# KangWelly/Assignment-for-AAE6102_GNSS-SDR

Measured on NVIDIA B200. Metric: search cells/s (PRN x Doppler x code-phase), 32-PRN acquisition, higher is better.
Workload: dtype f32

## Files before the change

### assignment-for-aae6102_gnss-sdr_b200/csrc/gnss_engine.h

```cpp
#pragma once
#include "gnss_radix.h"

#if defined(__CUDACC__)
#include <cuda_runtime.h>
#else
#include <cmath>
#endif

namespace gnss {

template <int Q>
struct Geo {
    static constexpr int N = 2000 * Q;
    static constexpr int ROW = 125 * Q;
    static constexpr int NX = 16 * (2 * Q - 1) * 125;
    static constexpr int M1 = 125 * Q, M2 = 16 * Q, M3 = 2000;
    static constexpr int INV1 = cmodinv(M1 % 16, 16);
    static constexpr int INV2 = cmodinv(M2 % 125, 125);
    static constexpr int INV3 = cmodinv(M3 % Q, Q);
    static constexpr int E1 = M1 * INV1, E2 = M2 * INV2, E3 = M3 * INV3;
    static_assert(Q % 2 == 1 && Q % 5 != 0, "Q must be coprime to 2000");
    static_assert(INV1 && INV2 && INV3, "no modular inverse");

    GNSS_HD static int good(int a, int b, int c) { return (a * M1 + b * M2 + c * M3) % N; }
// ... 193 lines not shown
    using X = GeoX<Q>;
    const int al = task / (5 * Q);
    const cf* p = D + task * 25 + al * (S::RS - S::ROW);
    cf v[25];
    static_for<0, 25>([&](auto ic) {
        constexpr int I = decltype(ic)::value;
        v[I] = p[I];
    });
    dft25(v);
    cf* q = xrow0 + al * X::RSX + (task - al * X::NT);
    static_for<0, 25>([&](auto ic) {
        constexpr int I = decltype(ic)::value;
        q[I * X::NTP] = v[5 * (I % 5) + I / 5];
    });
}
template <int Q, int R, class Storer>
GNSS_HD void pass4_task_xt(int j, int rank, const cf* __restrict__ X, Storer& st) {
    using GX = GeoX<Q>;
    using SX = SplitX<Q, R>;
    const int t = 2 * j;
    const int e = rank * SX::CHX + t;
    if (t >= SX::CHX || e >= GX::RSX) return;
    cf w0[16], w1[16];
    static_for<0, 16>([&](auto ac) {
        constexpr int Aidx = decltype(ac)::value;
        const cf2 v = ld_cg2(reinterpret_cast<const cf2*>(X + Aidx * GX::RSX + e));
        w0[Aidx] = v.lo;
        w1[Aidx] = v.hi;
    });
    dft16(w0);
    dft16(w1);
    st.template store2x<Q, R>(t, w0, w1);
}

template <int Q, int R, class Storer>
GNSS_HD void pass4_task(int j, int rank, cf* const* Dall, Storer& st) {
    using S = Split<Q, R>;
    const int t = 2 * j;
    const int col = rank * S::CH + t;
    if (t >= S::CH || col >= S::ROW) return;
    cf w0[16], w1[16];
    static_for<0, 16>([&](auto ac) {
        constexpr int Aidx = decltype(ac)::value;
        const cf2 v = *reinterpret_cast<const cf2*>(Dall[Aidx / S::A] + (Aidx % S::A) * S::RS + col);
        w0[Aidx] = v.lo;
        w1[Aidx] = v.hi;
    });
// ... 91 lines not shown
};

struct RegAccumStorer {
    float (&a0)[16];
    float (&a1)[16];
    template <int Q, int R>
    GNSS_HD void store2x(int , const cf (&w0)[16], const cf (&w1)[16]) {
        static_for<0, 16>([&](auto i_) {
            constexpr int I = decltype(i_)::value;
            constexpr int AP = (I / 4) + 4 * (I % 4);
            a0[AP] = cnorm_acc(w0[I], a0[AP]);
            a1[AP] = cnorm_acc(w1[I], a1[AP]);
        });
    }
};

struct SpectrumStorer {
    cf* __restrict__ out;
    float scale;
    int conj;
    int extended;
    template <int Q, int R>
    GNSS_HD void store1(int col, const cf (&w)[16]) {
        using G = Geo<Q>;
        const int cp = col / 125, pos = col - cp * 125;
        const int bp = G::bprime_of_pos(pos);
        const int bg = (bp * G::INV2) % 125, cg = (cp * G::INV3) % Q;
        const int planes = extended ? 2 * Q - 1 : Q;
        static_for<0, 16>([&](auto i_) {
            constexpr int I = decltype(i_)::value;
// ... 149 lines not shown
```

### assignment-for-aae6102_gnss-sdr_b200/csrc/gnss_internal.h

```cpp
#pragma once
#include <cuda_runtime.h>
#include <cstddef>
#include <cstdint>
#include "gnss_engine.h"

namespace gnss {

struct Candidate {
    float peak;
    int lag;
    double sum_all;
    double sum_win;
};

struct SearchArgs {
    const cf* cc;
    const cf* x;
    const int* bin_base;
    const int* bin_shift;
    int P, B, K;
    int row_first, n_rows;
    int w;
    Candidate* cand;
    int cand_stride;
    float* surface;
    cf* scratch;
    unsigned* group_ctr;
    Candidate* row_slots;
    float* partial;
    unsigned* part_ctr;
    unsigned* row_ticket;
    int row_granular;
#ifdef GNSS_TIMELINE
    unsigned long long* timeline;
#endif
};

struct WipeArgs {
    const void* raw;
    int data_type, precision, coh_ms, K;
    size_t block_bytes;
    const double* base_freq_hz;
    double fs_hz;
    const double* means;
    cf* x;
};

// ... 56 lines not shown
```

### assignment-for-aae6102_gnss-sdr_b200/csrc/gnss_kernels.cuh

```cuda
#pragma once
#include <cooperative_groups.h>
#include <climits>
#include "gnss_internal.h"

namespace gnss {
namespace cg = cooperative_groups;

struct NaturalLoader {
    static constexpr bool kStreams = false;
    const cf* __restrict__ in;
    template <int Q>
    __device__ __forceinline__ void load(int a, int b, cf (&z)[Q]) const {
        static_for<0, Q>([&](auto c_) {
            constexpr int C = decltype(c_)::value;
            z[C] = in[Geo<Q>::good(a, b, C)];
        });
    }
};
struct NaturalStorer {
    cf* __restrict__ out;
    template <int Q, int R>
    __device__ __forceinline__ void store2(int col, int, const cf (&w0)[16], const cf (&w1)[16]) {
        static_for<0, 16>([&](auto i_) {
            constexpr int I = decltype(i_)::value;
// ... 516 lines not shown
        }
        if constexpr (R > 1) cluster.sync(); else __syncthreads();
    }
}

__device__ __forceinline__ void group_arrive(unsigned* ctr) {
#ifdef GNSS_EXPERIMENT_NOFENCE
    asm volatile("red.relaxed.gpu.global.add.u32 [%0], 1;" ::"l"(ctr) : "memory");
#else
    asm volatile("red.release.gpu.global.add.u32 [%0], 1;" ::"l"(ctr) : "memory");
#endif
}
__device__ __forceinline__ void group_arrive_n(unsigned* ctr, unsigned n) {
    asm volatile("red.release.gpu.global.add.u32 [%0], %1;" ::"l"(ctr), "r"(n) : "memory");
}
__device__ __forceinline__ void group_spin(const unsigned* ctr, unsigned target) {
    unsigned v;
    do {
        asm volatile("ld.acquire.gpu.global.u32 %0, [%1];" : "=r"(v) : "l"(ctr) : "memory");
    } while ((int)(v - target) < 0);
}

template <int Q, int R, int T>
__device__ __noinline__ void publish_plane(float* acc, float* dst, int tid) {
    using SX = SplitX<Q, R>;
    for (int j = tid; j < SX::P4_TASKS; j += T) {
#pragma unroll
        for (int ap = 0; ap < 16; ++ap) {
            float2* p = reinterpret_cast<float2*>(acc + ap * SX::CHX + 2 * j);
            __stcg(reinterpret_cast<float2*>(dst + ap * SX::CHX + 2 * j), *p);
            *p = make_float2(0.f, 0.f);
        }
    }
}
template <int Q, int R, int T>
__device__ __noinline__ void merge_planes(float* acc, const float* planes, int n_planes, int tid) {
// ... 42 lines not shown
    using SX = SplitX<Q, R>;
    const int tid = threadIdx.x;
    const int tid2 = (tid + T - 32) % T;
    const int tid3 = (tid + T - (64 % T)) % T;
    const int rank = blockIdx.x % R, group = blockIdx.x / R, ngroups = gridDim.x / R;
    extern __shared__ __align__(16) unsigned char smem_raw[];
    cf* D = reinterpret_cast<cf*>(smem_raw);
    float* acc = reinterpret_cast<float*>(D + S::D_ELEMS);
    Tw4* tw = reinterpret_cast<Tw4*>(acc + Smem<Q, R>::acc_floats);
    RedScratch* rs = reinterpret_cast<RedScratch*>(tw + 100);
    constexpr size_t XBUF = (size_t)16 * GX::RSX;
    cf* xch = a.scratch + (size_t)group * 2 * XBUF;
    unsigned* ctr = a.group_ctr + group;
    Candidate* slots = a.row_slots + (size_t)group * R;
    unsigned target = 0;
    fill_tw125(tw, tid, T);
    constexpr bool kRoomy = (T * MINB <= 512);
    constexpr bool kRegAcc = (Q <= 13) && kRoomy && (SX::P4_TASKS <= T);
    float racc0[16], racc1[16];
#pragma unroll
    for (int q = 0; q < 16; ++q) { racc0[q] = 0.f; racc1[q] = 0.f; }
    RegAccumStorer rst{racc0, racc1};
    PowerAccumStorer st{acc};
    auto dump_acc = [&]() {
        if constexpr (kRegAcc) {
            if (tid < SX::P4_TASKS) {
#pragma unroll
                for (int ap = 0; ap < 16; ++ap) {
                    *reinterpret_cast<float2*>(acc + ap * SX::CHX + 2 * tid) = make_float2(racc0[ap], racc1[ap]);
                    racc0[ap] = 0.f; racc1[ap] = 0.f;
                }
            }
        }
    };
    const int n_rows = a.n_rows;
    auto loader_of = [&](int lrow) {
        const int row = a.row_first + lrow;
        const int p = row % a.P, b = row / a.P;
        int sa, sb, sc;
        G::shift_coords(a.bin_shift[b], sa, sb, sc);
        return SearchLoader{a.cc + (size_t)p * G::N, a.x + (size_t)a.bin_base[b] * a.K * G::NX, sa, sb, sc};
    };
    const int full = n_rows / ngroups, tail_base = full * ngroups, n_tail = n_rows - tail_base;
    auto tb = [&](int g) -> int {
        return a.row_granular ? (g < n_tail ? g : n_tail) * a.K : (int)((unsigned)g * (unsigned)(n_tail * a.K) / (unsigned)ngroups);
    };
    struct Part { int row, kb, ke; };
    auto part = [&](int i) -> Part {
        if (i < full) return Part{i * ngroups + group, 0, a.K};
        const int t0 = tb(group), t1 = tb(group + 1), r0 = t0 / a.K, e0 = min(t1, (r0 + 1) * a.K);
        if (i == full) return Part{tail_base + r0, t0 - r0 * a.K, e0 - r0 * a.K};
        return Part{tail_base + r0 + 1, 0, t1 - e0};
    };
    auto count_parts = [&]() -> int {
        const int t0 = tb(group), t1 = tb(group + 1);
        return full + (t0 < t1 ? 1 + (min(t1, (t0 / a.K + 1) * a.K) < t1) : 0);
    };
    if (count_parts() == 0) return;
    int i = 0, par = 0;
    const Part first = part(0);
    int left = first.ke - first.kb;
    bool later = first.kb > 0;
    for (int e = tid; e < SX::ACC_ELEMS; e += T) acc[e] = 0.f;
    SearchLoader ld = loader_of(first.row);
    ld.x += (size_t)first.kb * G::NX;
    for (int t = tid; t < S::P1_TASKS; t += T) pass1_task<Q, R>(t, rank, ld, D);
    __syncthreads();
    pass2_all<Q, R, T>(D, tw, tid2);
    __syncthreads();
    for (int t = tid3; t < S::P3_TASKS; t += T) pass3_task_xt<Q, R>(t, D, xch + (size_t)rank * S::A * GX::RSX);
#ifdef GNSS_TIMELINE
    int tl_iter = 0;
#endif
    for (;;) {
#ifdef GNSS_TIMELINE
        ++tl_iter;
#endif
        GNSS_TL(0);
        const bool last_of_part = (left == 1);
        const bool more = !last_of_part || i + 1 < count_parts();
        const cf* buf = xch + (size_t)par * XBUF;
        cf* nbuf = xch + (size_t)(par ^ 1) * XBUF;
        par ^= 1;
        target += R;
        if (more) {
            if (last_of_part) {
                const Part np = part(i + 1);
                ld = loader_of(np.row);
                ld.x += (size_t)np.kb * G::NX;
            } else {
                ld.x += G::NX;
            }
            cf z[Q];
            const bool has = tid < S::P1_TASKS;
            if (has) pass1_compute<Q, R>(tid, rank, ld, z);
            constexpr bool kTwo = (Q <= 13) && kRoomy && (S::P1_TASKS > T) && (S::P1_TASKS <= 2 * T);
            cf z2[kTwo ? Q : 1];
            const bool has2 = kTwo && tid + T < S::P1_TASKS;
            if constexpr (kTwo) { if (has2) pass1_compute<Q, R>(tid + T, rank, ld, z2); }
            GNSS_TL(1);
            GNSS_KSYNC();
            GNSS_TL(2);
            if (tid == 0) group_arrive(ctr);
            GNSS_TL(3);
            if (has) pass1_store<Q, R>(tid, z, D);
            if constexpr (kTwo) {
                if (has2) pass1_store<Q, R>(tid + T, z2, D);
            } else if constexpr (S::P1_TASKS > T) {
                for (int t = tid + T; t < S::P1_TASKS; t += T) pass1_task<Q, R>(t, rank, ld, D);
            }
            GNSS_TL(4);
            GNSS_KSYNC();
            GNSS_TL(5);
            pass2_all<Q, R, T>(D, tw, tid2);
            GNSS_TL(6);
        } else {
            GNSS_KSYNC();
            if (tid == 0) group_arrive(ctr);
        }
#ifndef GNSS_EXPERIMENT_NOSPIN
        if (tid == 0) group_spin(ctr, target);
#endif
        GNSS_TL(7);
        GNSS_KSYNC();
        GNSS_TL(8);
#pragma unroll 1
        for (int half = 0; half < 2; ++half) {
            const int flip = (((tid >> 5) + 1) >> 1) & 1;
            if ((half ^ flip) == 0) {
                if constexpr (kRegAcc) {
                    if (tid < SX::P4_TASKS) pass4_task_xt<Q, R>(tid, rank, buf, rst);
                } else {
                    for (int t = tid; t < SX::P4_TASKS; t += T) pass4_task_xt<Q, R>(t, rank, buf, st);
                }
            } else if (more) {
                for (int t = tid3; t < S::P3_TASKS; t += T) pass3_task_xt<Q, R>(t, D, nbuf + (size_t)rank * S::A * GX::RSX);
            }
        }
        GNSS_TL(10);
        if (later) {
            const Part cp = part(i);
            const int kk = cp.ke - left;
            int gf = group - 1;
            while (tb(gf) > (cp.row - tail_base) * a.K) --gf;
            float* dst = a.partial + (((size_t)gf * (a.K - 1) + (kk - 1)) * R + rank) * SX::ACC_ELEMS;
            dump_acc();
            publish_plane<Q, R, T>(acc, dst, tid);
            if (last_of_part) {
                __syncthreads();
                if (tid == 0) group_arrive_n(a.part_ctr + (size_t)gf * R + rank, (unsigned)(cp.ke - cp.kb));
            }
        } else if (last_of_part) {
            dump_acc();
            __syncthreads();
            const Part cp = part(i);
            const int row = cp.row;
            if (cp.ke < a.K) {
                if (tid == 0) group_spin(a.part_ctr + (size_t)group * R + rank, (unsigned)(a.K - cp.ke));
                __syncthreads();
                merge_planes<Q, R, T>(acc, a.partial + (((size_t)group * (a.K - 1) + (cp.ke - 1)) * R + rank) * SX::ACC_ELEMS,
                                      a.K - cp.ke, tid);
                __syncthreads();
            }
            const int p = (a.row_first + row) % a.P, b = (a.row_first + row) / a.P;
            float bv = -1.f;
            int bm = INT_MAX;
            double ss = 0.0;
            if (a.surface) {
                for (int e = tid; e < SX::ACC_ELEMS; e += T) {
                    const int ap = e / SX::CHX, t = e - ap * SX::CHX;
                    const int ex = rank * SX::CHX + t;
                    if (GX::valid(ex)) {
                        const float v = acc[e];
                        const int m = GX::lag_of(ap, ex);
// ... 17 lines not shown
                            const int ex = rank * SX::CHX + t;
                            if (vv[u] >= bv && GX::valid(ex)) {
                                const int m = GX::lag_of(ap, ex);
                                if (peak_better(vv[u], m, bv, bm)) { bv = vv[u]; bm = m; }
                            }
                        }
                    }
                }
            }
            block_reduce<T>(bv, bm, ss, rs);
            target += R;
            if (tid == 0) {
                Candidate c; c.peak = bv; c.lag = bm; c.sum_all = ss; c.sum_win = 0.0;
                slots[rank] = c;
                group_arrive(ctr);
                group_spin(ctr, target);
                float gv = -1.f;
                int gm = INT_MAX;
                for (int r = 0; r < R; ++r) {
                    const float ov = __ldcg(&slots[r].peak);
                    const int om = __ldcg(&slots[r].lag);
                    if (peak_better(ov, om, gv, gm)) { gv = ov; gm = om; }
                }
                rs->g_peak = gv;
                rs->g_lag = gm;
            }
            __syncthreads();
            const int gm = rs->g_lag;
            double wsum = 0.0;
            for (int i = tid; i < 2 * a.w - 1; i += T) {
                const int m = gm - (a.w - 1) + i;
                if (m >= 0 && m < G::N) {
                    int ap, ex;
                    GX::cell_of_lag(m, ap, ex);
                    if (ex / SX::CHX == rank) {
                        const float v = acc[ap * SX::CHX + (ex - rank * SX::CHX)];
                        wsum += (double)v * (double)v;
                    }
                }
            }
            float dv = -1.f;
            int dm = INT_MAX;
            block_reduce<T>(dv, dm, wsum, rs);
            if constexpr (!kRegAcc)
                for (int e = tid; e < SX::ACC_ELEMS; e += T) acc[e] = 0.f;
            if (tid == 0) {
                slots[rank].sum_win = wsum;
                unsigned old;
                asm volatile("atom.acq_rel.gpu.global.add.u32 %0, [%1], 1;" : "=r"(old) : "l"(a.row_ticket + group) : "memory");
                if ((old + 1) % R == 0) {
                    double s_all = 0.0, s_win = 0.0;
                    for (int r = 0; r < R; ++r) {
                        s_all += __ldcg(&slots[r].sum_all);
                        s_win += __ldcg(&slots[r].sum_win);
                    }
                    Candidate c;
                    c.peak = rs->g_peak;
                    c.lag = rs->g_lag;
                    c.sum_all = s_all;
                    c.sum_win = s_win;
                    a.cand[(size_t)p * a.cand_stride + b] = c;
                }
            }
        }
        if (!more) break;
        if (last_of_part) {
            const Part np = part(++i);
            left = np.ke - np.kb;
            later = np.kb > 0;
        } else {
            --left;
        }
    }
}

template <class K, class A>
static cudaError_t launch_clustered(K kern, const A& args, int units, int R, int T, size_t smem, cudaStream_t s) {
    cudaLaunchConfig_t cfg = {};
    cfg.gridDim = dim3((unsigned)(units * R), 1, 1);
    cfg.blockDim = dim3((unsigned)T, 1, 1);
    cfg.dynamicSmemBytes = smem;
    cfg.stream = s;
    cudaLaunchAttribute attr[1];
    attr[0].id = cudaLaunchAttributeClusterDimension;
    attr[0].val.clusterDim.x = (unsigned)R;
    attr[0].val.clusterDim.y = 1;
    attr[0].val.clusterDim.z = 1;
    cfg.attrs = attr;
// ... 19 lines not shown
        if (e != cudaSuccess) return e;
        e = cudaFuncSetAttribute(fine_kernel<Q, RT, TT, MT>, cudaFuncAttributeMaxDynamicSharedMemorySize, (int)Smem<Q, RT>::transform);
        if (e != cudaSuccess) return e;
        e = cudaFuncSetAttribute(search_kernel_coop<Q, R, T, MINB>, cudaFuncAttributeMaxDynamicSharedMemorySize, (int)Smem<Q, R>::search);
        if (e != cudaSuccess) return e;

        e = cudaFuncSetAttribute(search_kernel_l2x<Q, R, T, MINB>, cudaFuncAttributeMaxDynamicSharedMemorySize, (int)Smem<Q, R>::search);
        if (e != cudaSuccess) return e;
        return cudaFuncSetAttribute(search_kernel<Q, R, T, MINB>, cudaFuncAttributeMaxDynamicSharedMemorySize, (int)Smem<Q, R>::search);
    }
    static cudaError_t launch_search_l2x(const SearchArgs& a, int clusters, cudaStream_t s) {
        if (R > 8) return cudaErrorInvalidConfiguration;
        return launch_clustered(search_kernel_l2x<Q, R, T, MINB>, a, clusters, R, T, Smem<Q, R>::search, s);
    }
    static cudaError_t launch_search_coop(const SearchArgs& a, int groups, cudaStream_t s) {
        SearchArgs copy = a;
        void* args[] = {&copy};
        return cudaLaunchCooperativeKernel((const void*)search_kernel_coop<Q, R, T, MINB>, dim3((unsigned)(groups * R)),
                                           dim3((unsigned)T), args, Smem<Q, R>::search, s);
    }
    static int max_groups_coop() {
        int per_sm = 0, dev = 0, sms = 0;
        if (cudaOccupancyMaxActiveBlocksPerMultiprocessor(&per_sm, search_kernel_coop<Q, R, T, MINB>, T, Smem<Q, R>::search) != cudaSuccess) { cudaGetLastError(); return 0; }
        cudaGetDevice(&dev);
        cudaDeviceGetAttribute(&sms, cudaDevAttrMultiProcessorCount, dev);
        return per_sm * sms / R;
    }
    static int max_clusters_l2x() {
        cudaLaunchConfig_t cfg = {};
        cfg.gridDim = dim3((unsigned)(R * 1024), 1, 1);
        cfg.blockDim = dim3((unsigned)T, 1, 1);
        cfg.dynamicSmemBytes = Smem<Q, R>::search;
        cudaLaunchAttribute attr[1];
        attr[0].id = cudaLaunchAttributeClusterDimension;
        attr[0].val.clusterDim.x = (unsigned)R;
        attr[0].val.clusterDim.y = 1;
        attr[0].val.clusterDim.z = 1;
        cfg.attrs = attr;
        cfg.numAttrs = 1;
        int n = 0;
// ... 37 lines not shown
```

### assignment-for-aae6102_gnss-sdr_b200/csrc/gnssacq.cu

```cuda
#include <algorithm>
#include <climits>
#include <cmath>
#include <cstdio>
#include <cstdlib>
#include <chrono>
#include <cstring>
#include <string>
#include <vector>
#include <cooperative_groups.h>
#if defined(__x86_64__)
#include <emmintrin.h>
#endif

#include "../../include/gnssacq.h"
#include "gnss_internal.h"

using namespace gnss;

#define GNSSACQ_VERSION_STR "gnssacq 0.2.0 (sm_100a)"

namespace {

thread_local std::string g_create_error;

// ... 505 lines not shown
    int8_t* d_scode = nullptr;
    cf* d_cc = nullptr;
    cf* d_x = nullptr;
    int *d_bin_base = nullptr, *d_bin_shift = nullptr, *d_prn = nullptr;
    double* d_base_freq = nullptr;
    double* d_base_w = nullptr;
    unsigned char* d_comb = nullptr;
    int comb_pitch = 0;
    Candidate* d_cand = nullptr;
    gnssacq_result* d_res = nullptr;
    float* d_surface = nullptr;
    cf* d_scratch = nullptr;
    int l2x_clusters = 0;
    int coop_groups = 0;
    unsigned* d_group_ctr = nullptr;
    int bin0 = 0, B_full = 0;
    int row0 = 0, n_rows = 0;
    struct Xchg {
        bool on = false, is_root = false;
        gnssacq_shard sh{};
        unsigned char* block = nullptr;
        bool ipc_opened = false;
        unsigned char* if_buf = nullptr;
        Candidate* cand_all = nullptr;
        unsigned* flags = nullptr;
        int* d_prn_all = nullptr;
        gnssacq_result* d_res_all = nullptr;
        gnssacq_result* h_res_all = nullptr;
        unsigned epoch = 0;
        cudaEvent_t ev_a = nullptr, ev_b = nullptr, ev_c = nullptr, ev_d = nullptr;
// ... 33 lines not shown
    gnssacq_result* h_res = nullptr;
    cudaEvent_t ev[6] = {};
    cudaEvent_t ev_upload = nullptr;
    bool have_h2d = false;
    int launches = 0;
    std::string err;
};

namespace {

int fail(gnssacq_handle* h, int code, const std::string& msg) {
    if (h) h->err = msg;
    g_create_error = msg;
    return code;
}
#define CU(call)                                                                                         \
    do {                                                                                                 \
        cudaError_t e__ = (call);                                                                        \
        if (e__ != cudaSuccess)                                                                          \
            return fail(h, GNSSACQ_ERR_CUDA, std::string(#call) + ": " + cudaGetErrorString(e__));       \
    } while (0)

const VariantOps* pick_variant(int Q, int R, int T) {
    int n = 0;
    const VariantOps* v = nullptr;
    if (Q == 3) v = gnss_variants_q3(&n);
    else if (Q == 13) v = gnss_variants_q13(&n);
    else if (Q == 29) v = gnss_variants_q29(&n);
    if (!v) return nullptr;
    for (int i = 0; i < n; ++i)
// ... 116 lines not shown
        for (cudaEvent_t e : {h->xc.ev_a, h->xc.ev_b, h->xc.ev_c, h->xc.ev_d}) if (e) cudaEventDestroy(e);
    }
    if (h->ev_upload) cudaEventDestroy(h->ev_upload);
    if (h->h_if2) cudaFreeHost(h->h_if2);
    if (h->copy_stream) cudaStreamDestroy(h->copy_stream);
    for (auto& e : h->ev_copied) if (e) cudaEventDestroy(e);
    for (auto& e : h->ev_consumed) if (e) cudaEventDestroy(e);
    cudaFree(h->d_sums); cudaFree(h->d_means);
    cudaFree(h->d_trk_raw); cudaFree(h->d_trk_ca); cudaFree(h->d_trk_ch); cudaFree(h->d_trk_spacing); cudaFree(h->d_trk_partial);
    cudaFree(h->d_trk_out); cudaFree(h->d_trk_mean); cudaFree(h->d_trk_rec); cudaFree(h->d_trk_status);
    if (h->h_trk_out) cudaFreeHost(h->h_trk_out);
    cudaFree(h->d_fft_in); cudaFree(h->d_fft_out);
    cudaFree(h->d_fine_raw); cudaFree(h->d_fine_chip); cudaFree(h->d_fine_u); cudaFree(h->d_fine_ca); cudaFree(h->d_fine_start); cudaFree(h->d_fine_best);
    if (h->h_if) cudaFreeHost(h->h_if);
    if (h->h_res) cudaFreeHost(h->h_res);
    for (auto& e : h->ev) if (e) cudaEventDestroy(e);
    if (h->own_stream) cudaStreamDestroy(h->own_stream);
    delete h;
    return GNSSACQ_OK;
}

int gnssacq_create(const gnssacq_config* cfg, gnssacq_handle** out) {
    gnssacq_handle* h = nullptr;
    if (!out) return fail(nullptr, GNSSACQ_ERR_INVALID_ARG, "out is NULL");
    *out = nullptr;
    std::string why;
    int rc = validate(cfg, why);
    if (rc != GNSSACQ_OK) return fail(nullptr, rc, why);

    const int Q = cfg->samples_per_ms / 2000;
// ... 84 lines not shown
            const long long rows = h->n_rows, rounds = (rows + n - 1) / n;
            by_blocks = (double)(rounds * n - rows) >= 0.04 * (double)(rounds * n);
        }
        const long long max_useful = by_blocks ? (long long)h->n_rows * h->K : (long long)h->n_rows;
        if (n > max_useful) n = (int)max_useful;
        if (n <= 0) {
            gnssacq_destroy(h);
            return fail(nullptr, GNSSACQ_ERR_CUDA, "persistent search kernel cannot be made resident on this device");
        }
        if (xmode == 3) h->coop_groups = n; else h->l2x_clusters = n;
        CUC(cudaMalloc(&h->d_scratch, (size_t)n * ops->scratch_bytes_per_cluster));
        CUC(cudaMemsetAsync(h->d_scratch, 0, (size_t)n * ops->scratch_bytes_per_cluster, h->stream));
        CUC(cudaMalloc(&h->d_group_ctr, (size_t)n * (2 + ops->R) * sizeof(unsigned)));
        if (by_blocks) CUC(cudaMalloc(&h->d_partial, (size_t)n * (h->K - 1) * ops->partial_bytes_per_group));
        CUC(cudaMalloc(&h->d_row_slots, (size_t)n * ops->R * sizeof(Candidate)));
    }
    if (cfg->keep_surface) {
        CUC(cudaMalloc(&h->d_surface, (size_t)h->P * h->B * N * sizeof(float)));
        if (h->n_rows < h->P * h->B) CUC(cudaMemset(h->d_surface, 0, (size_t)h->P * h->B * N * sizeof(float)));
    }
    CUC(cudaMallocHost(&h->h_if, h->if_bytes));
    CUC(cudaMallocHost(&h->h_res, h->P * sizeof(gnssacq_result)));
    CUC(cudaMemcpyAsync(h->d_bin_base, h->bin_base.data(), h->B * sizeof(int), cudaMemcpyHostToDevice, h->stream));
    CUC(cudaMemcpyAsync(h->d_bin_shift, h->bin_shift.data(), h->B * sizeof(int), cudaMemcpyHostToDevice, h->stream));
    CUC(cudaMemcpyAsync(h->d_prn, cfg->prn, h->P * sizeof(int), cudaMemcpyHostToDevice, h->stream));
    CUC(cudaMemcpyAsync(h->d_base_freq, h->base_freq.data(), nb * sizeof(double), cudaMemcpyHostToDevice, h->stream));
    if (h->n_rows < h->P * h->B) {
        std::vector<Candidate> none((size_t)h->P * h->B, Candidate{-1.f, 0, 0.0, 0.0});
        CUC(cudaMemcpyAsync(h->d_cand, none.data(), none.size() * sizeof(Candidate), cudaMemcpyHostToDevice, h->stream));
        CUC(cudaStreamSynchronize(h->stream));
// ... 137 lines not shown
    sa.bin_base = h->d_bin_base;
    sa.bin_shift = h->d_bin_shift;
    sa.P = h->P; sa.B = h->B; sa.K = h->K;
    sa.row_first = h->row0; sa.n_rows = h->n_rows;
    sa.w = h->w;
    sa.cand = xchg ? xc.cand_all + (size_t)xc.sh.prn_first * xc.sh.freq_num_total + xc.sh.bin_first : h->d_cand;
    sa.cand_stride = xchg ? xc.sh.freq_num_total : h->B;
    sa.surface = h->d_surface;
    sa.scratch = h->d_scratch;
    sa.group_ctr = h->d_group_ctr;
    sa.row_slots = h->d_row_slots;
    sa.partial = h->d_partial;
    sa.part_ctr = h->d_group_ctr ? h->d_group_ctr + h->coop_groups : nullptr;
    sa.row_ticket = h->d_group_ctr ? h->d_group_ctr + (size_t)h->coop_groups * (1 + h->ops->R) : nullptr;
    sa.row_granular = h->d_partial ? 0 : 1;
#ifdef GNSS_TIMELINE
    static unsigned long long* d_timeline = nullptr;
    if (!d_timeline) { CU(cudaMalloc(&d_timeline, 16 * 16 * 32 * sizeof(unsigned long long))); }
    CU(cudaMemsetAsync(d_timeline, 0, 16 * 16 * 32 * sizeof(unsigned long long), s));
    sa.timeline = d_timeline;
    g_timeline = d_timeline;
#endif
    if (h->coop_groups > 0) {
        CU(cudaMemsetAsync(h->d_group_ctr, 0, (size_t)h->coop_groups * (2 + h->ops->R) * sizeof(unsigned), s));
        CU(h->ops->launch_search_coop(sa, h->coop_groups, s));
    } else if (h->l2x_clusters > 0) {
        CU(h->ops->launch_search_l2x(sa, h->l2x_clusters, s));
    } else {
        CU(h->ops->launch_search(sa, h->n_rows, s));
    }
    h->launches += 1;
    CU(cudaEventRecord(h->ev[3], s));
    if (xchg) {
        if (!xc.is_root) {
            xchg_done_kernel<<<1, 1, 0, s>>>(xc.flags + 1 + xc.sh.rank, xc.epoch);
            CU(cudaGetLastError());
            h->launches += 1;
        }
        CU(cudaEventRecord(h->ev[4], s));
        return GNSSACQ_OK;
// ... 21 lines not shown
    if (!h || !d_if || !d_out_rows) return fail(h, GNSSACQ_ERR_INVALID_ARG, "NULL argument");
    if (nbytes < h->if_bytes) return fail(h, GNSSACQ_ERR_SHORT_BUFFER, "IF block shorter than noncoh_blocks*coh_ms ms");
    CU(cudaSetDevice(h->device));
    h->have_h2d = false;
    CU(cudaEventRecord(h->ev[0], h->stream));
    return enqueue(h, d_if, (gnssacq_result*)d_out_rows);
}

int gnssacq_fetch_results(gnssacq_handle* h, gnssacq_result* out, gnssacq_stats* st) {
    if (!h || (!out && !st)) return fail(h, GNSSACQ_ERR_INVALID_ARG, "NULL argument");
    if (!h->d_last_rows) return fail(h, GNSSACQ_ERR_STATE, "no search has been enqueued on this handle");
    CU(cudaSetDevice(h->device));
    if (out) CU(cudaMemcpyAsync(h->h_res, h->d_last_rows, h->P * sizeof(gnssacq_result), cudaMemcpyDeviceToHost, h->stream));
    CU(cudaEventRecord(h->ev[5], h->stream));
    CU(cudaStreamSynchronize(h->stream));
    if (out) std::memcpy(out, h->h_res, h->P * sizeof(gnssacq_result));
    if (st) {
        std::memset(st, 0, sizeof(*st));
        if (h->have_h2d) cudaEventElapsedTime(&st->h2d_ms, h->ev[0], h->ev[1]);
        cudaEventElapsedTime(&st->wipeoff_fft_ms, h->ev[1], h->ev[2]);
        cudaEventElapsedTime(&st->search_ms, h->ev[2], h->ev[3]);
        cudaEventElapsedTime(&st->finalize_ms, h->ev[3], h->ev[4]);
        cudaEventElapsedTime(&st->d2h_ms, h->ev[4], h->ev[5]);
        cudaEventElapsedTime(&st->total_ms, h->ev[0], h->ev[5]);
        st->kernel_launches = h->launches;
        st->n_bases = (int)h->base_freq.size();
        st->cluster_ctas = h->ops->R;
        st->threads = h->ops->T;
        st->exchange = h->coop_groups > 0 ? 3 : (h->l2x_clusters > 0 ? 2 : 1);
        st->resident_clusters = h->coop_groups > 0 ? h->coop_groups : h->l2x_clusters;
// ... 202 lines not shown
    h->launches += 1;
    CU(cudaEventRecord(h->ev[4], s));
    return GNSSACQ_OK;
}

int gnssacq_xchg_fetch(gnssacq_handle* h, gnssacq_result* out, gnssacq_stats* st) {
    if (!h || !h->xc.on) return fail(h, GNSSACQ_ERR_STATE, "no exchange set up on this handle");
    if (out && !h->xc.is_root) return fail(h, GNSSACQ_ERR_INVALID_ARG, "rows are on the root");
    CU(cudaSetDevice(h->device));
    auto& xc = h->xc;
    const int n = xc.sh.n_prn_total;
    unsigned timed_out = 0;
    if (xc.is_root && out) CU(cudaMemcpyAsync(xc.h_res_all, xc.d_res_all, n * sizeof(gnssacq_result), cudaMemcpyDeviceToHost, h->stream));
    CU(cudaEventRecord(h->ev[5], h->stream));
    CU(cudaStreamSynchronize(h->stream));
    if (xc.is_root) {
        CU(cudaMemcpy(&timed_out, xc.flags + 63, sizeof timed_out, cudaMemcpyDeviceToHost));
        if (timed_out) return fail(h, GNSSACQ_ERR_STATE, "a shard of the exchange did not answer within the time-out");
        if (out) std::memcpy(out, xc.h_res_all, n * sizeof(gnssacq_result));
    }
    if (st) {
        std::memset(st, 0, sizeof(*st));
        if (h->have_h2d) cudaEventElapsedTime(&st->h2d_ms, h->ev[0], h->ev[1]);
        cudaEventElapsedTime(&st->wipeoff_fft_ms, h->ev[1], h->ev[2]);
        cudaEventElapsedTime(&st->search_ms, h->ev[2], h->ev[3]);
        if (xc.is_root) {
            if (cudaEventElapsedTime(&st->gather_wait_ms, xc.ev_c, xc.ev_d) != cudaSuccess) st->gather_wait_ms = 0.f;
            if (cudaEventElapsedTime(&st->finalize_ms, xc.ev_d, h->ev[4]) != cudaSuccess) st->finalize_ms = 0.f;
            cudaEventElapsedTime(&st->d2h_ms, h->ev[4], h->ev[5]);
        } else {
// ... 83 lines not shown
        if (i >= 2) CU(cudaStreamWaitEvent(h->copy_stream, h->ev_consumed[b], 0));
        else if (i == 0) CU(cudaStreamWaitEvent(h->copy_stream, h->ev[4], 0));
        CU(cudaMemcpyAsync(d_buf[b], h_buf[b], h->if_bytes, cudaMemcpyHostToDevice, h->copy_stream));
        CU(cudaEventRecord(h->ev_copied[b], h->copy_stream));
        CU(cudaStreamWaitEvent(h->stream, h->ev_copied[b], 0));
        h->have_h2d = false;
        CU(cudaEventRecord(h->ev[0], h->stream));
        int rc = enqueue(h, d_buf[b], h->d_res_sweep + (size_t)i * h->P);
        if (rc != GNSSACQ_OK) return rc;
        launches += h->launches;
        CU(cudaEventRecord(h->ev_consumed[b], h->stream));
    }
    CU(cudaMemcpyAsync(out, h->d_res_sweep, (size_t)n_windows * h->P * sizeof(gnssacq_result), cudaMemcpyDeviceToHost, h->stream));
    CU(cudaEventRecord(h->ev[5], h->stream));
    CU(cudaStreamSynchronize(h->stream));
    if (st) {
        std::memset(st, 0, sizeof(*st));
        st->total_ms = std::chrono::duration<float, std::milli>(std::chrono::steady_clock::now() - t0).count();
        cudaEventElapsedTime(&st->wipeoff_fft_ms, h->ev[1], h->ev[2]);
        cudaEventElapsedTime(&st->search_ms, h->ev[2], h->ev[3]);
        cudaEventElapsedTime(&st->finalize_ms, h->ev[3], h->ev[4]);
        st->kernel_launches = launches;
        st->n_bases = (int)h->base_freq.size();
        st->cluster_ctas = h->ops->R;
        st->threads = h->ops->T;
        st->exchange = h->coop_groups > 0 ? 3 : (h->l2x_clusters > 0 ? 2 : 1);
        st->resident_clusters = h->coop_groups > 0 ? h->coop_groups : h->l2x_clusters;
        st->work_split = h->d_partial ? 2 : 1;
    }
    return GNSSACQ_OK;
// ... 338 lines not shown
```

Baseline: 10.77 billion.

## Stage code strips and power accumulators in Blackwell tensor memory for cooperative search

The cooperative search kernel now allocates tensor memory (tcgen05) per CTA. It stages each thread's replica-code strip there once per row and reuses it across blocks instead of reloading the code from global memory. The non-register accumulator path keeps its power sums in tensor memory rather than in the shared-memory acc array. The launch also moves from cudaLaunchCooperativeKernel to a plain launch with a hand-computed residency limit that includes TMEM columns, and adds a spin timeout plus a mapped-host error flag so a stalled group gives up. A per-device event orders coop searches. The risks are extra TMEM load/store latency, tighter occupancy, and reliance on co-residency without the cooperative launch guarantee.

```diff
diff --git a/assignment-for-aae6102_gnss-sdr_b200/csrc/gnss_engine.h b/assignment-for-aae6102_gnss-sdr_b200/csrc/gnss_engine.h
--- a/assignment-for-aae6102_gnss-sdr_b200/csrc/gnss_engine.h
+++ b/assignment-for-aae6102_gnss-sdr_b200/csrc/gnss_engine.h
@@ -231,14 +231,13 @@
         q[I * X::NTP] = v[5 * (I % 5) + I / 5];
     });
 }
-template <int Q, int R, class Storer>
-GNSS_HD void pass4_task_xt(int j, int rank, const cf* __restrict__ X, Storer& st) {
+template <int Q, int R>
+GNSS_HD bool pass4_xt_dft(int j, int rank, const cf* __restrict__ X, cf (&w0)[16], cf (&w1)[16]) {
     using GX = GeoX<Q>;
     using SX = SplitX<Q, R>;
     const int t = 2 * j;
     const int e = rank * SX::CHX + t;
-    if (t >= SX::CHX || e >= GX::RSX) return;
-    cf w0[16], w1[16];
+    if (t >= SX::CHX || e >= GX::RSX) return false;
     static_for<0, 16>([&](auto ac) {
         constexpr int Aidx = decltype(ac)::value;
         const cf2 v = ld_cg2(reinterpret_cast<const cf2*>(X + Aidx * GX::RSX + e));
@@ -247,7 +246,13 @@
     });
     dft16(w0);
     dft16(w1);
-    st.template store2x<Q, R>(t, w0, w1);
+    return true;
+}
+template <int Q, int R, class Storer>
+GNSS_HD void pass4_task_xt(int j, int rank, const cf* __restrict__ X, Storer& st) {
+    cf w0[16], w1[16];
+    if (!pass4_xt_dft<Q, R>(j, rank, X, w0, w1)) return;
+    st.template store2x<Q, R>(2 * j, w0, w1);
 }
 
 template <int Q, int R, class Storer>
@@ -369,6 +374,139 @@
         });
     }
 };
+
+#if defined(__CUDACC__)
+__device__ __forceinline__ void tmem_ld2(uint32_t a, float (&v)[2]) {
+    asm volatile("tcgen05.ld.sync.aligned.32x32b.x2.b32 {%0, %1}, [%2];" : "=f"(v[0]), "=f"(v[1]) : "r"(a));
+}
+__device__ __forceinline__ void tmem_ld4(uint32_t a, float (&v)[4]) {
+    asm volatile("tcgen05.ld.sync.aligned.32x32b.x4.b32 {%0, %1, %2, %3}, [%4];"
+                 : "=f"(v[0]), "=f"(v[1]), "=f"(v[2]), "=f"(v[3]) : "r"(a));
+}
+__device__ __forceinline__ void tmem_ld8(uint32_t a, float (&v)[8]) {
+    asm volatile("tcgen05.ld.sync.aligned.32x32b.x8.b32 {%0, %1, %2, %3, %4, %5, %6, %7}, [%8];"
+                 : "=f"(v[0]), "=f"(v[1]), "=f"(v[2]), "=f"(v[3]), "=f"(v[4]), "=f"(v[5]), "=f"(v[6]), "=f"(v[7]) : "r"(a));
+}
+__device__ __forceinline__ void tmem_wait_ld(float (&u)[2], float (&v)[4]) {
+    asm volatile("tcgen05.wait::ld.sync.aligned;" : "+f"(u[0]), "+f"(u[1]), "+f"(v[0]), "+f"(v[1]), "+f"(v[2]), "+f"(v[3]));
+}
+__device__ __forceinline__ void tmem_wait_ld(float (&v)[4]) {
+    asm volatile("tcgen05.wait::ld.sync.aligned;" : "+f"(v[0]), "+f"(v[1]), "+f"(v[2]), "+f"(v[3]));
+}
+__device__ __forceinline__ void tmem_wait_ld(float (&v)[8]) {
+    asm volatile("tcgen05.wait::ld.sync.aligned;"
+                 : "+f"(v[0]), "+f"(v[1]), "+f"(v[2]), "+f"(v[3]), "+f"(v[4]), "+f"(v[5]), "+f"(v[6]), "+f"(v[7]));
+}
+__device__ __forceinline__ void tmem_st2(uint32_t a, float x, float y) {
+    asm volatile("tcgen05.st.sync.aligned.32x32b.x2.b32 [%0], {%1, %2};" ::"r"(a), "f"(x), "f"(y));
+}
+__device__ __forceinline__ void tmem_st4(uint32_t a, cf p, cf q) {
+    asm volatile("tcgen05.st.sync.aligned.32x32b.x4.b32 [%0], {%1, %2, %3, %4};" ::"r"(a), "f"(p.x), "f"(p.y), "f"(q.x), "f"(q.y));
+}
+__device__ __forceinline__ void tmem_st8(uint32_t a, const float (&v)[8]) {
+    asm volatile("tcgen05.st.sync.aligned.32x32b.x8.b32 [%0], {%1, %2, %3, %4, %5, %6, %7, %8};"
+                 ::"r"(a), "f"(v[0]), "f"(v[1]), "f"(v[2]), "f"(v[3]), "f"(v[4]), "f"(v[5]), "f"(v[6]), "f"(v[7]));
+}
+__device__ __forceinline__ void tmem_wait_st() { asm volatile("tcgen05.wait::st.sync.aligned;"); }
+
+template <int Q>
+struct Strip {
+    static constexpr int COLS = 2 * Q + 2;
+};
+template <int Q, int R>
+__device__ __forceinline__ void strip_fill(const SearchLoader& ld, int task, int rank, uint32_t strip) {
+    const int al = task / 125, b = task - al * 125;
+    const cf* pc = ld.begin<Q>(rank * Split<Q, R>::A + al, b).pc;
+    const cf c0 = ld_ro(pc);
+    tmem_st2(strip, c0.x, c0.y);
+    static_for<1, (Q - 1) / 2 + 1>([&](auto jc) {
+        constexpr int J = decltype(jc)::value;
+        tmem_st4(strip + 4 * J, ld_ro(pc + J * 125), ld_ro(pc + (Q - J) * 125));
+    });
+}
+struct TmemSearchLoader {
+    static constexpr bool kStreams = true;
+    SearchLoader g;
+    uint32_t strip;
+    struct Ctx {
+        const cf* px;
+        uint32_t strip;
+        mutable float c0[2], cur[4], nxt[4];
+    };
+    template <int Q>
+    __device__ __forceinline__ Ctx begin(int a, int b) const {
+        Ctx c;
+        c.px = g.begin<Q>(a, b).px;
+        c.strip = strip;
+        tmem_ld2(strip, c.c0);
+        tmem_ld4(strip + 4, c.nxt);
+        tmem_wait_ld(c.c0, c.nxt);
+        return c;
+    }
+    template <int Q, int C>
+    __device__ __forceinline__ cf at(const Ctx& c) const {
+        constexpr int H = (Q - 1) / 2;
+        const cf x = ld_ro(c.px + C * 125);
+        if constexpr (C == 0) {
+            return cmul_scalar(mk(c.c0[0], c.c0[1]), x);
+        } else if constexpr (C <= H) {
+            if constexpr (C > 1) tmem_wait_ld(c.nxt);
+#pragma unroll
+            for (int i = 0; i < 4; ++i) c.cur[i] = c.nxt[i];
+            if constexpr (C < H) tmem_ld4(c.strip + 4 * (C + 1), c.nxt);
+            return cmul_scalar(mk(c.cur[0], c.cur[1]), x);
+        } else {
+            return cmul_scalar(mk(c.cur[2], c.cur[3]), x);
+        }
+    }
+};
+
+struct TmemAccumStorer {
+    uint32_t col;
+    bool has;
+    template <int Q, int R>
+    __device__ __forceinline__ void store2x(int , const cf (&w0)[16], const cf (&w1)[16]) const {
+        tmem_wait_st();
+        float v[8];
+        tmem_ld8(col, v);
+        static_for<0, 4>([&](auto c_) {
+            constexpr int C = decltype(c_)::value;
+            tmem_wait_ld(v);
+            float u[8];
+#pragma unroll
+            for (int i = 0; i < 8; ++i) u[i] = v[i];
+            if constexpr (C < 3) tmem_ld8(col + 8 * (C + 1), v);
+            if (has) {
+                static_for<0, 4>([&](auto i_) {
+                    constexpr int i = decltype(i_)::value, I = 4 * C + i;
+                    u[2 * i] = cnorm_acc(w0[I], u[2 * i]);
+                    u[2 * i + 1] = cnorm_acc(w1[I], u[2 * i + 1]);
+                });
+            }
+            tmem_st8(col + 8 * C, u);
+        });
+    }
+    template <int Q, int R>
+    __device__ __forceinline__ void dump(float* dst) const {
+        constexpr int CHX = SplitX<Q, R>::CHX;
+        constexpr float zero[8] = {0.f, 0.f, 0.f, 0.f, 0.f, 0.f, 0.f, 0.f};
+        tmem_wait_st();
+        static_for<0, 4>([&](auto c_) {
+            constexpr int C = decltype(c_)::value;
+            float v[8];
+            tmem_ld8(col + 8 * C, v);
+            tmem_wait_ld(v);
+            if (has) {
+                static_for<0, 4>([&](auto i_) {
+                    constexpr int i = decltype(i_)::value, I = 4 * C + i, AP = (I / 4) + 4 * (I % 4);
+                    *reinterpret_cast<float2*>(dst + AP * CHX) = make_float2(v[2 * i], v[2 * i + 1]);
+                });
+            }
+            tmem_st8(col + 8 * C, zero);
+        });
+    }
+};
+#endif
 
 struct SpectrumStorer {
     cf* __restrict__ out;
diff --git a/assignment-for-aae6102_gnss-sdr_b200/csrc/gnss_internal.h b/assignment-for-aae6102_gnss-sdr_b200/csrc/gnss_internal.h
--- a/assignment-for-aae6102_gnss-sdr_b200/csrc/gnss_internal.h
+++ b/assignment-for-aae6102_gnss-sdr_b200/csrc/gnss_internal.h
@@ -31,6 +31,7 @@
     unsigned* part_ctr;
     unsigned* row_ticket;
     int row_granular;
+    unsigned* error;
 #ifdef GNSS_TIMELINE
     unsigned long long* timeline;
 #endif
diff --git a/assignment-for-aae6102_gnss-sdr_b200/csrc/gnss_kernels.cuh b/assignment-for-aae6102_gnss-sdr_b200/csrc/gnss_kernels.cuh
--- a/assignment-for-aae6102_gnss-sdr_b200/csrc/gnss_kernels.cuh
+++ b/assignment-for-aae6102_gnss-sdr_b200/csrc/gnss_kernels.cuh
@@ -1,5 +1,6 @@
 #pragma once
 #include <cooperative_groups.h>
+#include <algorithm>
 #include <climits>
 #include "gnss_internal.h"
 
@@ -554,12 +555,33 @@
 __device__ __forceinline__ void group_arrive_n(unsigned* ctr, unsigned n) {
     asm volatile("red.release.gpu.global.add.u32 [%0], %1;" ::"l"(ctr), "r"(n) : "memory");
 }
-__device__ __forceinline__ void group_spin(const unsigned* ctr, unsigned target) {
+__device__ __forceinline__ bool group_spin(const unsigned* ctr, unsigned target) {
     unsigned v;
-    do {
+    long long t0 = 0;
+    for (;;) {
         asm volatile("ld.acquire.gpu.global.u32 %0, [%1];" : "=r"(v) : "l"(ctr) : "memory");
-    } while ((int)(v - target) < 0);
-}
+        if ((int)(v - target) >= 0) return true;
+        const long long t = clock64();
+        if (t0 == 0) t0 = t;
+        else if (t - t0 > 8000000000ll) return false;
+    }
+}
+
+template <int Q, int R, int T, int MINB>
+struct CoopTmem {
+    using S = Split<Q, R>;
+    using SX = SplitX<Q, R>;
+    static constexpr bool kRoomy = (T * MINB <= 512);
+    static constexpr bool kRegAcc = (Q <= 13) && kRoomy && (SX::P4_TASKS <= T);
+    static constexpr int ROUNDS = (S::P1_TASKS + T - 1) / T;
+    static constexpr int ACC = kRegAcc ? 0 : 32;
+    static constexpr int SET = (ACC + ROUNDS * Strip<Q>::COLS + 7) / 8 * 8;
+    static constexpr int USED = (T / 128) * SET;
+    static constexpr int COLS = USED <= 32 ? 32 : USED <= 64 ? 64 : USED <= 128 ? 128 : USED <= 256 ? 256 : 512;
+    static_assert(T % 128 == 0, "tensor-memory lanes: whole sets of 128 threads");
+    static_assert(SX::P4_TASKS <= T, "at most one pass-4 task per thread");
+    static_assert(USED <= 512, "tensor memory holds 512 columns per SM");
+};
 
 template <int Q, int R, int T>
 __device__ __noinline__ void publish_plane(float* acc, float* dst, int tid) {
@@ -632,14 +654,18 @@
     unsigned* ctr = a.group_ctr + group;
     Candidate* slots = a.row_slots + (size_t)group * R;
     unsigned target = 0;
+    using TM = CoopTmem<Q, R, T, MINB>;
+    __shared__ uint32_t tmem_base;
+    __shared__ int gave_up;
     fill_tw125(tw, tid, T);
-    constexpr bool kRoomy = (T * MINB <= 512);
-    constexpr bool kRegAcc = (Q <= 13) && kRoomy && (SX::P4_TASKS <= T);
-    float racc0[16], racc1[16];
+    constexpr bool kRoomy = TM::kRoomy;
+    constexpr bool kRegAcc = TM::kRegAcc;
+    float racc0[kRegAcc ? 16 : 1], racc1[kRegAcc ? 16 : 1];
+    if constexpr (kRegAcc) {
 #pragma unroll
-    for (int q = 0; q < 16; ++q) { racc0[q] = 0.f; racc1[q] = 0.f; }
-    RegAccumStorer rst{racc0, racc1};
-    PowerAccumStorer st{acc};
+        for (int q = 0; q < 16; ++q) { racc0[q] = 0.f; racc1[q] = 0.f; }
+    }
+    uint32_t tacc = 0, tstrip = 0;
     auto dump_acc = [&]() {
         if constexpr (kRegAcc) {
             if (tid < SX::P4_TASKS) {
@@ -649,7 +675,23 @@
                     racc0[ap] = 0.f; racc1[ap] = 0.f;
                 }
             }
-        }
+        } else {
+            TmemAccumStorer{tacc, tid < SX::P4_TASKS}.template dump<Q, R>(acc + 2 * tid);
+        }
+    };
+    auto give_up = [&]() {
+        *reinterpret_cast<volatile unsigned*>(a.error) = 1u;
+        __threadfence_system();
+        gave_up = 1;
+    };
+    auto task_of = [&](int k) { return min(tid + k * T, S::P1_TASKS - 1); };
+    auto fill_strips = [&](const SearchLoader& l) {
+#pragma unroll 1
+        for (int k = 0; k < TM::ROUNDS; ++k) strip_fill<Q, R>(l, task_of(k), rank, tstrip + k * Strip<Q>::COLS);
+        tmem_wait_st();
+    };
+    auto p1_compute = [&](const SearchLoader& l, int k, cf (&z)[Q]) {
+        pass1_compute<Q, R>(task_of(k), rank, TmemSearchLoader{l, tstrip + (uint32_t)(k * Strip<Q>::COLS)}, z);
     };
     const int n_rows = a.n_rows;
     auto loader_of = [&](int lrow) {
@@ -675,6 +717,17 @@
         return full + (t0 < t1 ? 1 + (min(t1, (t0 / a.K + 1) * a.K) < t1) : 0);
     };
     if (count_parts() == 0) return;
+    if (tid < 32) {
+        const unsigned slot = (unsigned)__cvta_generic_to_shared(&tmem_base);
+        asm volatile("tcgen05.alloc.cta_group::1.sync.aligned.shared::cta.b32 [%0], %1;" ::"r"(slot), "n"(TM::COLS) : "memory");
+        asm volatile("tcgen05.relinquish_alloc_permit.cta_group::1.sync.aligned;" ::: "memory");
+    }
+    if (tid == 0) gave_up = 0;
+    asm volatile("tcgen05.fence::before_thread_sync;" ::: "memory");
+    __syncthreads();
+    asm volatile("tcgen05.fence::after_thread_sync;" ::: "memory");
+    tacc = tmem_base + ((uint32_t)(32 * ((tid >> 5) & 3)) << 16) + (uint32_t)((tid >> 7) * TM::SET);
+    tstrip = tacc + TM::ACC;
     int i = 0, par = 0;
     const Part first = part(0);
     int left = first.ke - first.kb;
@@ -682,7 +735,13 @@
     for (int e = tid; e < SX::ACC_ELEMS; e += T) acc[e] = 0.f;
     SearchLoader ld = loader_of(first.row);
     ld.x += (size_t)first.kb * G::NX;
-    for (int t = tid; t < S::P1_TASKS; t += T) pass1_task<Q, R>(t, rank, ld, D);
+    fill_strips(ld);
+#pragma unroll 1
+    for (int k = 0; k < TM::ROUNDS; ++k) {
+        cf z[Q];
+        p1_compute(ld, k, z);
+        if (tid + k * T < S::P1_TASKS) pass1_store<Q, R>(tid + k * T, z, D);
+    }
     __syncthreads();
     pass2_all<Q, R, T>(D, tw, tid2);
     __syncthreads();
@@ -706,16 +765,17 @@
                 const Part np = part(i + 1);
                 ld = loader_of(np.row);
                 ld.x += (size_t)np.kb * G::NX;
+                fill_strips(ld);
             } else {
                 ld.x += G::NX;
             }
             cf z[Q];
             const bool has = tid < S::P1_TASKS;
-            if (has) pass1_compute<Q, R>(tid, rank, ld, z);
+            p1_compute(ld, 0, z);
             constexpr bool kTwo = (Q <= 13) && kRoomy && (S::P1_TASKS > T) && (S::P1_TASKS <= 2 * T);
             cf z2[kTwo ? Q : 1];
             const bool has2 = kTwo && tid + T < S::P1_TASKS;
-            if constexpr (kTwo) { if (has2) pass1_compute<Q, R>(tid + T, rank, ld, z2); }
+            if constexpr (kTwo) p1_compute(ld, 1, z2);
             GNSS_TL(1);
             GNSS_KSYNC();
             GNSS_TL(2);
@@ -724,8 +784,13 @@
             if (has) pass1_store<Q, R>(tid, z, D);
             if constexpr (kTwo) {
                 if (has2) pass1_store<Q, R>(tid + T, z2, D);
-            } else if constexpr (S::P1_TASKS > T) {
-                for (int t = tid + T; t < S::P1_TASKS; t += T) pass1_task<Q, R>(t, rank, ld, D);
+            } else {
+#pragma unroll 1
+                for (int k = 1; k < TM::ROUNDS; ++k) {
+                    cf z3[Q];
+                    p1_compute(ld, k, z3);
+                    if (tid + k * T < S::P1_TASKS) pass1_store<Q, R>(tid + k * T, z3, D);
+                }
             }
             GNSS_TL(4);
             GNSS_KSYNC();
@@ -737,19 +802,24 @@
             if (tid == 0) group_arrive(ctr);
         }
 #ifndef GNSS_EXPERIMENT_NOSPIN
-        if (tid == 0) group_spin(ctr, target);
+        if (tid == 0 && !group_spin(ctr, target)) give_up();
 #endif
         GNSS_TL(7);
         GNSS_KSYNC();
         GNSS_TL(8);
+        if (gave_up) break;
 #pragma unroll 1
         for (int half = 0; half < 2; ++half) {
             const int flip = (((tid >> 5) + 1) >> 1) & 1;
             if ((half ^ flip) == 0) {
                 if constexpr (kRegAcc) {
+                    RegAccumStorer rst{racc0, racc1};
                     if (tid < SX::P4_TASKS) pass4_task_xt<Q, R>(tid, rank, buf, rst);
                 } else {
-                    for (int t = tid; t < SX::P4_TASKS; t += T) pass4_task_xt<Q, R>(t, rank, buf, st);
+                    cf w0[16], w1[16];
+                    const bool has4 = tid < SX::P4_TASKS && rank * SX::CHX + 2 * tid < GX::RSX;
+                    pass4_xt_dft<Q, R>(has4 ? tid : 0, has4 ? rank : 0, buf, w0, w1);
+                    TmemAccumStorer{tacc, has4}.template store2x<Q, R>(2 * tid, w0, w1);
                 }
             } else if (more) {
                 for (int t = tid3; t < S::P3_TASKS; t += T) pass3_task_xt<Q, R>(t, D, nbuf + (size_t)rank * S::A * GX::RSX);
@@ -774,8 +844,9 @@
             const Part cp = part(i);
             const int row = cp.row;
             if (cp.ke < a.K) {
-                if (tid == 0) group_spin(a.part_ctr + (size_t)group * R + rank, (unsigned)(a.K - cp.ke));
+                if (tid == 0 && !group_spin(a.part_ctr + (size_t)group * R + rank, (unsigned)(a.K - cp.ke))) give_up();
                 __syncthreads();
+                if (gave_up) break;
                 merge_planes<Q, R, T>(acc, a.partial + (((size_t)group * (a.K - 1) + (cp.ke - 1)) * R + rank) * SX::ACC_ELEMS,
                                       a.K - cp.ke, tid);
                 __syncthreads();
@@ -823,7 +894,7 @@
                 Candidate c; c.peak = bv; c.lag = bm; c.sum_all = ss; c.sum_win = 0.0;
                 slots[rank] = c;
                 group_arrive(ctr);
-                group_spin(ctr, target);
+                if (!group_spin(ctr, target)) give_up();
                 float gv = -1.f;
                 int gm = INT_MAX;
                 for (int r = 0; r < R; ++r) {
@@ -835,6 +906,7 @@
                 rs->g_lag = gm;
             }
             __syncthreads();
+            if (gave_up) break;
             const int gm = rs->g_lag;
             double wsum = 0.0;
             for (int i = tid; i < 2 * a.w - 1; i += T) {
@@ -851,8 +923,6 @@
             float dv = -1.f;
             int dm = INT_MAX;
             block_reduce<T>(dv, dm, wsum, rs);
-            if constexpr (!kRegAcc)
-                for (int e = tid; e < SX::ACC_ELEMS; e += T) acc[e] = 0.f;
             if (tid == 0) {
                 slots[rank].sum_win = wsum;
                 unsigned old;
@@ -881,6 +951,11 @@
             --left;
         }
     }
+    tmem_wait_st();
+    asm volatile("tcgen05.fence::before_thread_sync;" ::: "memory");
+    __syncthreads();
+    asm volatile("tcgen05.fence::after_thread_sync;" ::: "memory");
+    if (tid < 32) asm volatile("tcgen05.dealloc.cta_group::1.sync.aligned.b32 %0, %1;" ::"r"(tmem_base), "n"(TM::COLS) : "memory");
 }
 
 template <class K, class A>
@@ -930,16 +1005,25 @@
         return launch_clustered(search_kernel_l2x<Q, R, T, MINB>, a, clusters, R, T, Smem<Q, R>::search, s);
     }
     static cudaError_t launch_search_coop(const SearchArgs& a, int groups, cudaStream_t s) {
-        SearchArgs copy = a;
-        void* args[] = {&copy};
-        return cudaLaunchCooperativeKernel((const void*)search_kernel_coop<Q, R, T, MINB>, dim3((unsigned)(groups * R)),
-                                           dim3((unsigned)T), args, Smem<Q, R>::search, s);
+        search_kernel_coop<Q, R, T, MINB><<<(unsigned)(groups * R), (unsigned)T, Smem<Q, R>::search, s>>>(a);
+        return cudaGetLastError();
     }
     static int max_groups_coop() {
-        int per_sm = 0, dev = 0, sms = 0;
-        if (cudaOccupancyMaxActiveBlocksPerMultiprocessor(&per_sm, search_kernel_coop<Q, R, T, MINB>, T, Smem<Q, R>::search) != cudaSuccess) { cudaGetLastError(); return 0; }
-        cudaGetDevice(&dev);
-        cudaDeviceGetAttribute(&sms, cudaDevAttrMultiProcessorCount, dev);
+        cudaFuncAttributes fa;
+        if (cudaFuncGetAttributes(&fa, search_kernel_coop<Q, R, T, MINB>) != cudaSuccess) { cudaGetLastError(); return 0; }
+        int dev = 0, sms = 0, regs_sm = 0, smem_sm = 0, smem_rsv = 0, thr_sm = 0, blk_sm = 0;
+        if (cudaGetDevice(&dev) != cudaSuccess ||
+            cudaDeviceGetAttribute(&sms, cudaDevAttrMultiProcessorCount, dev) != cudaSuccess ||
+            cudaDeviceGetAttribute(&regs_sm, cudaDevAttrMaxRegistersPerMultiprocessor, dev) != cudaSuccess ||
+            cudaDeviceGetAttribute(&smem_sm, cudaDevAttrMaxSharedMemoryPerMultiprocessor, dev) != cudaSuccess ||
+            cudaDeviceGetAttribute(&smem_rsv, cudaDevAttrReservedSharedMemoryPerBlock, dev) != cudaSuccess ||
+            cudaDeviceGetAttribute(&thr_sm, cudaDevAttrMaxThreadsPerMultiProcessor, dev) != cudaSuccess ||
+            cudaDeviceGetAttribute(&blk_sm, cudaDevAttrMaxBlocksPerMultiprocessor, dev) != cudaSuccess) { cudaGetLastError(); return 0; }
+        const int regs_warp = (fa.numRegs * 32 + 255) / 256 * 256;
+        const int warps_by_regs = regs_warp > 0 ? (regs_sm / 4 / regs_warp) * 4 : INT_MAX;
+        const size_t smem_cta = fa.sharedSizeBytes + Smem<Q, R>::search + (size_t)smem_rsv;
+        const int per_sm = std::min({warps_by_regs / (T / 32), (int)((size_t)smem_sm / smem_cta), thr_sm / T, blk_sm,
+                               512 / CoopTmem<Q, R, T, MINB>::COLS});
         return per_sm * sms / R;
     }
     static int max_clusters_l2x() {
diff --git a/assignment-for-aae6102_gnss-sdr_b200/csrc/gnssacq.cu b/assignment-for-aae6102_gnss-sdr_b200/csrc/gnssacq.cu
--- a/assignment-for-aae6102_gnss-sdr_b200/csrc/gnssacq.cu
+++ b/assignment-for-aae6102_gnss-sdr_b200/csrc/gnssacq.cu
@@ -5,6 +5,8 @@
 #include <cstdlib>
 #include <chrono>
 #include <cstring>
+#include <map>
+#include <mutex>
 #include <string>
 #include <vector>
 #include <cooperative_groups.h>
@@ -543,6 +545,7 @@
     int l2x_clusters = 0;
     int coop_groups = 0;
     unsigned* d_group_ctr = nullptr;
+    unsigned* h_search_err = nullptr;
     int bin0 = 0, B_full = 0;
     int row0 = 0, n_rows = 0;
     struct Xchg {
@@ -606,6 +609,16 @@
     g_create_error = msg;
     return code;
 }
+
+int check_search_error(gnssacq_handle* h) {
+    if (!h->h_search_err || !*h->h_search_err) return GNSSACQ_OK;
+    *h->h_search_err = 0;
+    return fail(h, GNSSACQ_ERR_STATE, "the search kernel's CTA groups did not all meet within ~4 s (was the device shared "
+                                      "with other work?); the rows of that search are invalid");
+}
+
+std::mutex g_search_order_mu;
+std::map<int, cudaEvent_t> g_last_search;
 #define CU(call)                                                                                         \
     do {                                                                                                 \
         cudaError_t e__ = (call);                                                                        \
@@ -752,6 +765,7 @@
     cudaFree(h->d_fine_raw); cudaFree(h->d_fine_chip); cudaFree(h->d_fine_u); cudaFree(h->d_fine_ca); cudaFree(h->d_fine_start); cudaFree(h->d_fine_best);
     if (h->h_if) cudaFreeHost(h->h_if);
     if (h->h_res) cudaFreeHost(h->h_res);
+    if (h->h_search_err) cudaFreeHost(h->h_search_err);
     for (auto& e : h->ev) if (e) cudaEventDestroy(e);
     if (h->own_stream) cudaStreamDestroy(h->own_stream);
     delete h;
@@ -866,6 +880,10 @@
         CUC(cudaMalloc(&h->d_group_ctr, (size_t)n * (2 + ops->R) * sizeof(unsigned)));
         if (by_blocks) CUC(cudaMalloc(&h->d_partial, (size_t)n * (h->K - 1) * ops->partial_bytes_per_group));
         CUC(cudaMalloc(&h->d_row_slots, (size_t)n * ops->R * sizeof(Candidate)));
+        if (xmode == 3) {
+            CUC(cudaHostAlloc(&h->h_search_err, sizeof(unsigned), cudaHostAllocMapped));
+            *h->h_search_err = 0;
+        }
     }
     if (cfg->keep_surface) {
         CUC(cudaMalloc(&h->d_surface, (size_t)h->P * h->B * N * sizeof(float)));
@@ -1033,6 +1051,7 @@
     sa.part_ctr = h->d_group_ctr ? h->d_group_ctr + h->coop_groups : nullptr;
     sa.row_ticket = h->d_group_ctr ? h->d_group_ctr + (size_t)h->coop_groups * (1 + h->ops->R) : nullptr;
     sa.row_granular = h->d_partial ? 0 : 1;
+    sa.error = nullptr;
 #ifdef GNSS_TIMELINE
     static unsigned long long* d_timeline = nullptr;
     if (!d_timeline) { CU(cudaMalloc(&d_timeline, 16 * 16 * 32 * sizeof(unsigned long long))); }
@@ -1042,7 +1061,13 @@
 #endif
     if (h->coop_groups > 0) {
         CU(cudaMemsetAsync(h->d_group_ctr, 0, (size_t)h->coop_groups * (2 + h->ops->R) * sizeof(unsigned), s));
+        CU(cudaHostGetDevicePointer((void**)&sa.error, h->h_search_err, 0));
+        std::lock_guard<std::mutex> lock(g_search_order_mu);
+        cudaEvent_t& last = g_last_search[h->device];
+        if (!last) CU(cudaEventCreateWithFlags(&last, cudaEventDisableTiming));
+        else CU(cudaStreamWaitEvent(s, last, 0));
         CU(h->ops->launch_search_coop(sa, h->coop_groups, s));
+        CU(cudaEventRecord(last, s));
     } else if (h->l2x_clusters > 0) {
         CU(h->ops->launch_search_l2x(sa, h->l2x_clusters, s));
     } else {
@@ -1094,6 +1119,7 @@
     if (out) CU(cudaMemcpyAsync(h->h_res, h->d_last_rows, h->P * sizeof(gnssacq_result), cudaMemcpyDeviceToHost, h->stream));
     CU(cudaEventRecord(h->ev[5], h->stream));
     CU(cudaStreamSynchronize(h->stream));
+    if (int rc = check_search_error(h)) return rc;
     if (out) std::memcpy(out, h->h_res, h->P * sizeof(gnssacq_result));
     if (st) {
         std::memset(st, 0, sizeof(*st));
@@ -1326,6 +1352,7 @@
     if (xc.is_root && out) CU(cudaMemcpyAsync(xc.h_res_all, xc.d_res_all, n * sizeof(gnssacq_result), cudaMemcpyDeviceToHost, h->stream));
     CU(cudaEventRecord(h->ev[5], h->stream));
     CU(cudaStreamSynchronize(h->stream));
+    if (int rc = check_search_error(h)) return rc;
     if (xc.is_root) {
         CU(cudaMemcpy(&timed_out, xc.flags + 63, sizeof timed_out, cudaMemcpyDeviceToHost));
         if (timed_out) return fail(h, GNSSACQ_ERR_STATE, "a shard of the exchange did not answer within the time-out");
@@ -1439,6 +1466,7 @@
     CU(cudaMemcpyAsync(out, h->d_res_sweep, (size_t)n_windows * h->P * sizeof(gnssacq_result), cudaMemcpyDeviceToHost, h->stream));
     CU(cudaEventRecord(h->ev[5], h->stream));
     CU(cudaStreamSynchronize(h->stream));
+    if (int rc = check_search_error(h)) return rc;
     if (st) {
         std::memset(st, 0, sizeof(*st));
         st->total_ms = std::chrono::duration<float, std::milli>(std::chrono::steady_clock::now() - t0).count();
```

New measurement: 11.11 billion (median of 6 runs). +3.2%, better.
